# yifita/iso-points

Measured on AMD Instinct MI355X. Metric: Mpoints/s full iso-point cycle (project+resample+splat), 1M pts, higher is better.
Workload: dtype f32-class (split-fp16 operands, 2^-22: hidden-layer products from two fp16 parts per f32 operand under exact power-of-two scales, 3 fp16-MFMA passes, f32 accumulate; everything else f32)

## Files before the change

### include/isopoints.h

```cpp
#ifndef ISOPOINTS_H_
#define ISOPOINTS_H_

#include <stdint.h>

#ifdef __cplusplus
extern "C" {
#endif

#define ISO_OK 0
#define ISO_ERR_INVALID (-1)
#define ISO_ERR_UNSUPPORTED (-2)
#define ISO_ERR_LAUNCH (-3)
#define ISO_ERR_WORKSPACE (-4)

const char* iso_version(void);
const char* iso_last_error(void);


int iso_project_sphere(const float* pts_in, float* pts_out, float* normals_out,
                       uint8_t* mask_out, int64_t n, float cx, float cy,
                       float cz, float radius, int max_iters, float tol,
                       void* stream);

typedef struct iso_follow {
  void* grid_ws; int64_t grid_n_max;
  const float* views; int n_views; float znear; float zfar; int backface_culling;
  int32_t* mask_out; void* front_ws; int64_t front_ws_bytes;
  int64_t* first_idx_out; int64_t* num_pts_out; int32_t* view_total_out;
} iso_follow;

int iso_project_sphere_follow(const float* pts_in, float* pts_out, float* normals_out,
                              uint8_t* mask_out, int64_t n, float cx, float cy,
                              float cz, float radius, int max_iters, float tol,
                              const iso_follow* follow_host, void* stream);

int64_t iso_siren_raw_floats(int hidden, int n_hidden);
int64_t iso_siren_packed_floats(int hidden, int n_hidden);
int iso_siren_pack_weights(const float* raw, float* packed, int hidden,
                           int n_hidden, void* stream);
int iso_siren_set_gemm_mode(int mode);
int iso_siren_get_gemm_mode(void);
int iso_siren_set_tail_from(int first_tail_iteration);
int iso_siren_set_drawn_tiles(int on);
int iso_idr_set_drawn_tiles(int on);
int iso_siren_step_launches(int hidden, int n_hidden, int max_iters);
int64_t iso_project_siren_workspace_bytes(int64_t n, int hidden, int n_hidden);
int64_t iso_project_siren_counts_offset(int64_t n, int hidden, int n_hidden);
int iso_project_siren(const float* pts_in, float* pts_out, float* normals_out,
                      uint8_t* mask_out, int64_t n, const float* packed,
                      int hidden, int n_hidden, float omega_first,
                      float omega_hidden, int max_iters, float tol,
                      void* workspace, int64_t workspace_bytes, void* stream);
int iso_siren_sdf_grad(const float* pts, float* sdf_out, float* grad_out,
                       int64_t n, const float* packed, int hidden,
                       int n_hidden, float omega_first, float omega_hidden,
                       void* workspace, int64_t workspace_bytes, void* stream);

int iso_siren_fold_codes(const float* w0c, const float* b0, const float* codes, float* table, int hidden,
                         int padded_hidden, int c_dim, int64_t n_codes, void* stream);
int iso_project_siren_coded(const float* pts_in, float* pts_out, float* normals_out,
                            uint8_t* mask_out, int64_t n, const float* packed,
                            int hidden, int n_hidden, float omega_first,
                            float omega_hidden, int max_iters, float tol,
                            void* workspace, int64_t workspace_bytes, void* stream,
                            const float* code_bias, const int32_t* code_of, int64_t n_codes);
int iso_siren_sdf_grad_coded(const float* pts, float* sdf_out, float* grad_out,
                             int64_t n, const float* packed, int hidden,
                             int n_hidden, float omega_first, float omega_hidden,
                             void* workspace, int64_t workspace_bytes, void* stream,
                             const float* code_bias, const int32_t* code_of, int64_t n_codes);

int64_t iso_idr_raw_floats(int hidden, int n_layers, int skip_layer, int n_freq);
int64_t iso_idr_packed_floats(int hidden, int n_layers);
int iso_idr_pack_weights(const float* raw, float* packed, int hidden, int n_layers,
                         int skip_layer, int n_freq, void* stream);
int64_t iso_project_idr_workspace_bytes(int64_t n, int hidden, int n_layers);
int iso_project_idr(const float* pts_in, float* pts_out, float* normals_out, uint8_t* mask_out,
                    int64_t n, const float* packed, int hidden, int n_layers, int skip_layer,
                    int n_freq, float beta, int max_iters, float tol, void* workspace,
                    int64_t workspace_bytes, void* stream);
int iso_idr_sdf_grad(const float* pts, float* sdf_out, float* grad_out, int64_t n,
                     const float* packed, int hidden, int n_layers, int skip_layer, int n_freq,
                     float beta, void* workspace, int64_t workspace_bytes, void* stream);

int iso_trace_sphere(const float* ray0, const float* dirs, float* pts_out, float* sdf_out,
                     uint8_t* mask_out, int64_t n, float cx, float cy, float cz, float radius,
                     float alpha, float bound, int max_iters, float tol, void* stream);
int iso_trace_siren(const float* ray0, const float* dirs, float* pts_out, float* sdf_out,
                    uint8_t* mask_out, int64_t n, const float* packed, int hidden, int n_hidden,
                    float omega_first, float omega_hidden, float alpha, float bound, int max_iters,
                    float tol, void* workspace, int64_t workspace_bytes, void* stream);
int iso_trace_siren_coded(const float* ray0, const float* dirs, float* pts_out, float* sdf_out,
// ... 352 lines not shown
```

### iso_points_amd/_lib.py

```python
import ctypes
import os

import torch

_HERE = os.path.dirname(os.path.abspath(__file__))
LIB_PATH = os.path.join(_HERE, "libisopoints_hip.so")
if os.environ.get("ISO_DEV_LIB"):
    LIB_PATH = os.path.abspath(os.environ["ISO_DEV_LIB"])

_c = ctypes
_P = _c.c_void_p
_I = _c.c_int
_L = _c.c_int64
_F = _c.c_float

SIGNATURES = {
    "iso_version": (_c.c_char_p, []),
    "iso_last_error": (_c.c_char_p, []),
    "iso_project_sphere": (_I, [_P, _P, _P, _P, _L, _F, _F, _F, _F, _I, _F, _P]),
    "iso_project_sphere_follow": (_I, [_P, _P, _P, _P, _L, _F, _F, _F, _F, _I, _F, _P, _P]),
    "iso_siren_raw_floats": (_L, [_I, _I]),
    "iso_siren_packed_floats": (_L, [_I, _I]),
    "iso_siren_set_gemm_mode": (_I, [_I]),
    "iso_siren_get_gemm_mode": (_I, []),
    "iso_siren_set_tail_from": (_I, [_I]),
    "iso_siren_set_drawn_tiles": (_I, [_I]),
    "iso_idr_set_drawn_tiles": (_I, [_I]),
    "iso_siren_step_launches": (_I, [_I, _I, _I]),
    "iso_siren_pack_weights": (_I, [_P, _P, _I, _I, _P]),
    "iso_project_siren_workspace_bytes": (_L, [_L, _I, _I]),
    "iso_project_siren_counts_offset": (_L, [_L, _I, _I]),
    "iso_project_siren": (_I, [_P, _P, _P, _P, _L, _P, _I, _I, _F, _F, _I, _F, _P, _L, _P]),
    "iso_siren_sdf_grad": (_I, [_P, _P, _P, _L, _P, _I, _I, _F, _F, _P, _L, _P]),
    "iso_idr_raw_floats": (_L, [_I, _I, _I, _I]),
    "iso_idr_packed_floats": (_L, [_I, _I]),
    "iso_idr_pack_weights": (_I, [_P, _P, _I, _I, _I, _I, _P]),
    "iso_project_idr_workspace_bytes": (_L, [_L, _I, _I]),
    "iso_project_idr": (_I, [_P, _P, _P, _P, _L, _P, _I, _I, _I, _I, _F, _I, _F, _P, _L, _P]),
    "iso_idr_sdf_grad": (_I, [_P, _P, _P, _L, _P, _I, _I, _I, _I, _F, _P, _L, _P]),
    "iso_trace_sphere": (_I, [_P, _P, _P, _P, _P, _L, _F, _F, _F, _F, _F, _F, _I, _F, _P]),
    "iso_trace_siren": (_I, [_P, _P, _P, _P, _P, _L, _P, _I, _I, _F, _F, _F, _F, _I, _F, _P, _L, _P]),
    "iso_siren_fold_codes": (_I, [_P, _P, _P, _P, _I, _I, _I, _L, _P]),
    "iso_project_siren_coded": (_I, [_P, _P, _P, _P, _L, _P, _I, _I, _F, _F, _I, _F, _P, _L, _P, _P, _P, _L]),
    "iso_siren_sdf_grad_coded": (_I, [_P, _P, _P, _L, _P, _I, _I, _F, _F, _P, _L, _P, _P, _P, _L]),
    "iso_trace_siren_coded": (_I, [_P, _P, _P, _P, _P, _L, _P, _I, _I, _F, _F, _F, _F, _I, _F, _P, _L, _P, _P, _P, _L]),
    "iso_trace_idr": (_I, [_P, _P, _P, _P, _P, _L, _P, _I, _I, _I, _I, _F, _F, _F, _I, _F, _P, _L, _P]),
    "iso_ray_nearest_point_workspace_bytes": (_L, [_L]),
    "iso_ray_nearest_point": (_I, [_P, _L, _F, _F, _F, _P, _L, _P, _P, _P, _P, _L, _P]),
    "iso_raymarch_settle": (_I, [_P, _P, _L, _P, _P, _P, _P, _F, _I, _I, _P, _P, _P, _P]),
    "iso_raymarch_overshoot": (_I, [_P, _P, _L, _P, _P, _P, _P, _I, _I, _F, _P, _P, _P, _P]),
    "iso_raymarch_secant": (_I, [_P, _P, _L, _P, _P, _P, _P, _P, _P, _P, _P]),
    "iso_image_sample": (_I, [_P, _I, _I, _I, _I, _P, _L, _I, _P, _P]),
    "iso_ear_candidates": (_I, [_P, _P, _P, _P, _L, _I, _F, _P, _P, _P]),
    "iso_points_bbox": (_I, [_P, _P, _I, _L, _P, _P]),
    "iso_frnn_make_grid": (_I, [_P, _P, _P, _I, _L, _I, _P, _P]),
    "iso_frnn_make_grid_density": (_I, [_P, _P, _P, _I, _L, _I, _F, _P, _P]),
    "iso_frnn_insert_points": (_I, [_P, _P, _P, _P, _P, _P, _I, _L, _L, _I, _P]),
    "iso_prefix_sum_workspace_bytes": (_L, [_L, _I]),
    "iso_prefix_sum": (_I, [_P, _P, _L, _I, _L, _P, _L, _P]),
    "iso_frnn_scan_cells": (_I, [_P, _P, _P, _I, _L, _I, _P, _L, _P]),
    "iso_frnn_counting_sort": (_I, [_P, _P, _P, _P, _P, _P, _P, _I, _L, _L, _I, _P]),
    "iso_frnn_query_workspace_bytes": (_L, [_I, _L, _L]),
    "iso_frnn_query": (_I, [_P, _P, _P, _P, _P, _P, _P, _P, _P, _I, _P, _P, _P, _I, _L, _L, _L, _P, _L, _P]),
    "iso_frnn_gather": (_I, [_P, _P, _P, _I, _L, _L, _I, _I, _P]),
    "iso_repulse": (_I, [_P, _P, _P, _L, _P, _L, _L, _I, _P, _P]),
    "iso_upsample_candidates": (_I, [_P, _P, _L, _I, _P, _P, _P]),
    "iso_farthest_point_sampling_work_floats": (_L, [_I, _L]),
    "iso_farthest_point_sampling": (_I, [_P, _P, _P, _P, _I, _L, _L, _P, _P, _P]),
    "iso_pca_frames_work_bytes": (_L, [_I]),
    "iso_pca_frames": (_I, [_P, _P, _P, _I, _L, _I, _I, _P, _P, _P, _P]),
    "iso_splat_view_flags": (_I, [_P, _P, _P, _P, _L, _I, _F, _F, _I, _P]),
    "iso_compact_rows": (_I, [_P, _P, _P, _P, _L, _L, _I, _P]),
    "iso_splat_vrk_h": (_I, [_P, _P, _P, _P, _P, _I, _L, _P]),
    "iso_splat_setup": (_I, [_P, _P, _P, _P, _P, _P, _P, _I, _L, _I, _F, _F, _P, _P, _P, _P, _P, _P]),
    "iso_splat_vrk_h_global_work_bytes": (_L, [_I]),
    "iso_splat_vrk_h_global": (_I, [_P, _P, _P, _P, _I, _L, _L, _P, _P]),
    "iso_splat_tangent_frame": (_I, [_P, _L, _P, _P, _P]),
    "iso_splat_setup_vrk": (_I, [_P, _P, _P, _P, _P, _P, _P, _I, _L, _I, _F, _F, _P, _P, _P, _P, _P, _P]),
    "iso_splat_setup_aniso": (_I, [_P, _P, _L, _P, _P, _P, _P, _I, _I, _F, _F, _P, _P, _P, _P, _P, _P]),
    "iso_splat_tiles_per_side": (_I, [_I]),
    "iso_splat_bin_count": (_I, [_P, _P, _P, _P, _I, _L, _I, _I, _I, _I, _P, _P]),
    "iso_splat_tile_offsets": (_I, [_P, _P, _P, _L, _P]),
# ... 121 lines not shown
```

### iso_points_amd/csrc/siren.hip

```cpp
#include <stdlib.h>
#include "siren_common.h"
#include "iso_newton.h"
#include "mlp_common.h"

namespace {

__global__ void k_siren_pack(const float* __restrict__ raw, float* __restrict__ packed,
                             int H, int L) {
  const int64_t total = off_hidden(H, L);
  const int64_t HH = (int64_t)H * H;
  const int NT = H / 16;
  for (int64_t o = (int64_t)blockIdx.x * blockDim.x + threadIdx.x; o < total;
       o += (int64_t)gridDim.x * blockDim.x) {
    float v = 0.f;
    if (o < off_wl(H)) {
      int64_t k = o;
      int c = (int)(k & 3);
      int e = (int)((k >> 2) % (H / 4));
      int g = (int)((k >> 2) / (H / 4));
      int f = 16 * (e >> 2) + 4 * g + (e & 3);
      v = (c < 3) ? raw[f * 3 + c] : raw[(int64_t)H * 3 + f];
    } else if (o < off_bl(H)) {
      int64_t k = o - off_wl(H);
      int e = (int)(k % (H / 4));
      int g = (int)(k / (H / 4));
      int f = 16 * (e >> 2) + 4 * g + (e & 3);
      const int64_t raw_wl = (int64_t)H * 4 + (int64_t)L * (HH + H);
      v = raw[raw_wl + f];
    } else if (o < off_hidden(H, 0)) {
      const int64_t raw_wl = (int64_t)H * 4 + (int64_t)L * (HH + H);
      v = (o == off_bl(H)) ? raw[raw_wl + H] : 0.f;
    } else {
      int64_t k = o - off_hidden(H, 0);
      const int64_t per = H + 2 * HH;
      int l = (int)(k / per);
      int64_t w = k % per;
      const float* Wl = raw + (int64_t)H * 4 + (int64_t)l * (HH + H);
      const float* bl = Wl + HH;
      if (w < H) {
        v = bl[w];
      } else {
        w -= H;
        bool bwd = w >= HH;
        if (bwd) w -= HH;
        int i = (int)(w & 3);
        int lane = (int)((w >> 2) & 63);
        int t = (int)((w >> 8) % NT);
        int q = (int)((w >> 8) / NT);
        int a = 16 * t + (lane & 15);
        int b = 16 * q + 4 * (lane >> 4) + i;
        v = bwd ? Wl[(int64_t)b * H + a]
                : Wl[(int64_t)a * H + b];
      }
    }
    packed[o] = v;
  }
}

#define ISO_GEMM_FWD(img, bias) gemm_pass<NT, true>(img, bias, hL, wbuf, acc, lane, g)
#define ISO_GEMM_BWD(img) gemm_pass<NT, false>(img, nullptr, hL, wbuf, acc, lane, g)

template <int NT, bool CODED>
__global__ __launch_bounds__(256, 2) void k_siren_step(typename SirenArgsOf<CODED>::type a) {
  constexpr int H = NT * 16;
  extern __shared__ __attribute__((aligned(16))) float smem[];
  const int tid = threadIdx.x;
  const int wave = tid >> 6, lane = tid & 63;
  const int g = lane >> 4, j = lane & 15;
  float* hL = smem + wave * (NT * 256);
  float* wbuf = smem + 4 * NT * 256;
  const float* W0img = a.packed + off_w0(H);
  const float* WLimg = a.packed + off_wl(H);
  const float bL = a.packed[off_bl(H)];
  float* stash = a.stash + ((int64_t)blockIdx.x * 4 + wave) * (int64_t)(a.L + 1) * NT * 256;

  const int64_t count = a.count_in ? (int64_t)(*a.count_in) : a.n;
  const int64_t n_tiles = (count + 63) / 64;
  for (int64_t tile = blockIdx.x; tile < n_tiles; tile += gridDim.x) {
    const int64_t slot = tile * 64 + wave * 16 + j;
    const bool valid = slot < count;
    int64_t idx = -1;
    float px = 0.f, py = 0.f, pz = 0.f;
    int row = 0;
    if (valid) {
      idx = a.idx_in ? (int64_t)a.idx_in[slot] : slot;
      px = a.pts[idx * 3]; py = a.pts[idx * 3 + 1]; pz = a.pts[idx * 3 + 2];
      if constexpr (CODED) row = a.code_of ? a.code_of[idx] : 0;
    }
    const f32x4* cb = nullptr;
    if constexpr (CODED) cb = reinterpret_cast<const f32x4*>(a.code_bias + (int64_t)row * H) + g;
    (void)cb;
    float f = 0.f;
    const bool top0 = (a.L == 0);
    for (int e4 = 0; e4 < NT; ++e4) {
      f32x4 h4, s4;
      f32x4 b4 = {0.f, 0.f, 0.f, 0.f};
      if constexpr (CODED) b4 = cb[4 * e4];
#pragma unroll
      for (int i = 0; i < 4; ++i) {
        const f32x4 w = reinterpret_cast<const f32x4*>(W0img)[g * (H / 4) + e4 * 4 + i];
        float z;
        if constexpr (CODED) z = ((w.x * px + w.y * py) + w.z * pz) + b4[i];
        else z = ((w.x * px + w.y * py) + w.z * pz) + w.w;
        float s, c;
        iso_sincos(a.w0 * z, s, c);
        h4[i] = s;
        s4[i] = a.w0 * c;
      }
      if (top0) {
// ... 109 lines not shown
}

__global__ void k_zero_counts(int32_t* c, int n) {
  int i = blockIdx.x * blockDim.x + threadIdx.x;
  if (i < n) c[i] = 0;
}

bool siren_shape_ok(int H, int L) {
  return (H == 64 || H == 128 || H == 256) && L >= 0 && L <= 8;
}

int g_gemm_mode = -1;
int gemm_mode() {
  if (g_gemm_mode < 0) {
    const char* e = getenv("ISO_SIREN_GEMM");
    g_gemm_mode = (e && (!strcmp(e, "f32") || !strcmp(e, "0"))) ? 0 : 1;
  }
  return g_gemm_mode;
}
bool use_x3(int H, int L) { return gemm_mode() == 1 && siren_x3_supported(H, L); }

int64_t stash_floats_any(int H, int L) {
  int64_t a = stash_floats(H, L);
  int64_t b = siren_x3_supported(H, L) ? siren_x3_stash_floats(H, L) : 0;
  return a > b ? a : b;
}

int run_step(const SirenCodedArgs& a, int H, int64_t n, hipStream_t s) {
  if (use_x3(H, a.L)) return siren_x3_launch(a, H, n, s);
  int64_t tiles = (n + 63) / 64;
  int blocks = (int)(tiles < kSirenBlocks ? tiles : kSirenBlocks);
  return a.code_bias ? dispatch_step<true>(a, H, blocks, s) : dispatch_step<false>(a, H, blocks, s);
}

}

extern "C" int64_t iso_siren_raw_floats(int hidden, int n_hidden) {
  int64_t H = hidden;
  return H * 3 + H + (int64_t)n_hidden * (H * H + H) + H + 1;
}

extern "C" int64_t iso_siren_packed_floats(int hidden, int n_hidden) {
  return siren_packed_total(hidden, n_hidden);
}

extern "C" int iso_siren_set_gemm_mode(int mode) {
  ISO_REQUIRE(mode == 0 || mode == 1, ISO_ERR_INVALID, "iso_siren_set_gemm_mode: mode must be 0 (f32 MFMA) or 1 (split fp16)");
  g_gemm_mode = mode;
  return ISO_OK;
}

extern "C" int iso_siren_get_gemm_mode(void) { return gemm_mode(); }

extern "C" int iso_siren_pack_weights(const float* raw, float* packed, int hidden,
                                      int n_hidden, void* stream) {
  ISO_REQUIRE(siren_shape_ok(hidden, n_hidden), ISO_ERR_UNSUPPORTED,
              "iso_siren_pack_weights: hidden must be 64/128/256 and 0<=n_hidden<=8 (got %d, %d)",
              hidden, n_hidden);
  ISO_REQUIRE(raw && packed, ISO_ERR_INVALID, "iso_siren_pack_weights: null pointer");
  int64_t total = off_hidden(hidden, n_hidden);
  hipLaunchKernelGGL(k_siren_pack, dim3(iso_stream_grid(total, 256)), dim3(256), 0,
                     (hipStream_t)stream, raw, packed, hidden, n_hidden);
  if (hidden % 32 == 0) siren_x3_pack(raw, packed, hidden, n_hidden, (hipStream_t)stream);
  ISO_CHECK_LAUNCH("iso_siren_pack_weights");
  return ISO_OK;
}

static int64_t tail_cap_of(int64_t n) {
  const int64_t blocks = siren_x3_tail_blocks(), tiles = (n + 31) / 32;
  return ((tiles + blocks - 1) / blocks + 1) * 32;
}
static int64_t tail_ints(int64_t n) { return siren_x3_tail_blocks() * (2 * tail_cap_of(n) + 2); }

constexpr int kTileCtrInts = 128;
extern "C" int64_t iso_project_siren_workspace_bytes(int64_t n, int hidden, int n_hidden) {
  if (n < 0) n = 0;
  return stash_floats_any(hidden, n_hidden) * 4 + 2 * n * 4 + tail_ints(n) * 4 + (64 + kTileCtrInts) * 4 + 64;
}

extern "C" int64_t iso_project_siren_counts_offset(int64_t n, int hidden, int n_hidden) {
  if (n < 0) n = 0;
  return stash_floats_any(hidden, n_hidden) * 4 + 2 * n * 4 + tail_ints(n) * 4;
}

static int g_siren_dyn_tiles = -1;
static bool siren_dynamic_tiles_enabled() {
  return g_siren_dyn_tiles != 0;
}
extern "C" int iso_siren_set_drawn_tiles(int on) {
  ISO_REQUIRE(on >= -1 && on <= 1, ISO_ERR_INVALID, "iso_siren_set_drawn_tiles: -1 (default), 0 or 1");
  g_siren_dyn_tiles = on;
  return ISO_OK;
}

static int run_step_split(SirenCodedArgs a, int hidden, int64_t n, hipStream_t s) {
  if (hidden == 256 && !a.fwd_only && use_x3(hidden, a.L)) {
    a.split = 3;
    return run_step(a, hidden, n, s);
  }
  a.split = 0;
  a.tile_ctr = nullptr;
  return run_step(a, hidden, n, s);
}

static int g_tail_from = -1;
static int siren_tail_from(int max_iters) {
  if (g_tail_from == 0) return max_iters + 1;
  if (g_tail_from > 0) return g_tail_from;
  return max_iters >= 6 ? 4 : 2;
}
extern "C" int iso_siren_step_launches(int hidden, int n_hidden, int max_iters) {
  if (max_iters < 0) return 0;
  const bool can_tail = hidden == 256 && use_x3(hidden, n_hidden);
  const int from = can_tail ? siren_tail_from(max_iters) : max_iters + 1;
  return from <= max_iters && from > 0 ? from + 1 : max_iters + 1;
}
// ... 236 lines not shown
```

### iso_points_amd/csrc/siren_common.h

```cpp
#pragma once
#include "iso_common.h"

struct SirenArgs {
  float* pts;
  float* normals;
  uint8_t* mask;
  float* sdf_out;
  float* grad_out;
  const int32_t* idx_in;
  const int32_t* count_in;
  int32_t* idx_out;
  int32_t* count_out;
  const float* packed;
  float* stash;
  int64_t n;
  int L;
  float w0, wh, tol;
  int do_move;
  int eval_only;
  const float* dirs = nullptr;
  float alpha = 1.f, bound = 0.f, tol_valid = 0.f;
  int fwd_only = 0;
  int64_t cnt_lo = -1, cnt_hi = INT64_MAX;
  int small_tiles = 0;
  int split = 0;
  int big_blocks = 0;
  int32_t* tail_lists = nullptr;
  int32_t* tail_counts = nullptr;
  int32_t* iter_counts = nullptr;
  int tail_cap = 0, it_first = 0, it_last = 0;
  int32_t* tile_ctr = nullptr;
  int draw_first = 0;
  int ps_guard = 0;
};

struct SirenCodedArgs : SirenArgs {
  const float* code_bias = nullptr;
  const int32_t* code_of = nullptr;
};
template <bool CODED> struct SirenArgsOf { using type = SirenArgs; };
template <> struct SirenArgsOf<true> { using type = SirenCodedArgs; };

__host__ __device__ inline int64_t siren_split_point(int64_t count) {
  const int64_t big = 256 * 96, small = 256 * 32;
  const int64_t full = count / big * big, rem = count - full;
  if (rem == 0) return count;
  return (rem + small - 1) / small <= 2 ? full : count;
}

__host__ __device__ inline int64_t off_w0(int H) { (void)H; return 0; }
__host__ __device__ inline int64_t off_wl(int H) { return 4 * (int64_t)H; }
__host__ __device__ inline int64_t off_bl(int H) { return 5 * (int64_t)H; }
__host__ __device__ inline int64_t off_hidden(int H, int l) {
  return 5 * (int64_t)H + 4 + (int64_t)l * ((int64_t)H + 2 * (int64_t)H * H);
}

__host__ __device__ inline int x3_feat(int s, int kappa) {
  return 32 * (s >> 1) + 16 * (s & 1) + 8 * ((kappa & 7) >> 2) + 4 * (kappa >> 3) + (kappa & 3);
}
__host__ __device__ inline int64_t x3_base(int H, int L) { return off_hidden(H, L); }
__host__ __device__ inline int64_t x3_off_w0(int H, int L) { return x3_base(H, L); }
__host__ __device__ inline int64_t x3_off_wl(int H, int L) { return x3_base(H, L) + 4 * (int64_t)H; }
__host__ __device__ inline int64_t x3_off_layer(int H, int L, int l) {
  return x3_base(H, L) + 5 * (int64_t)H + (int64_t)l * (int64_t)H;
}
constexpr int kX16Header = 24;
__host__ __device__ inline int64_t x16_base(int H, int L) { return x3_off_layer(H, L, L); }
__host__ __device__ inline int64_t x16_off_layer(int H, int L, int l) { return x16_base(H, L) + kX16Header + (int64_t)l * H * H; }
__host__ __device__ inline int64_t x16_off_bw(int H, int L, int l) { return x16_off_layer(H, L, L) + (int64_t)l * H * H; }
__host__ __device__ inline int64_t siren_packed_total(int H, int L) { return x16_off_bw(H, L, L); }

bool siren_x3_supported(int H, int L);
int64_t siren_x3_stash_floats(int H, int L);
void siren_x3_pack(const float* raw, float* packed, int H, int L, hipStream_t s);
int siren_x3_launch(const SirenCodedArgs& a, int H, int64_t n_upper, hipStream_t s);
int siren_x3_tail_blocks();
int siren_x3_launch_tail(const SirenCodedArgs& a, int H, hipStream_t s);
constexpr int64_t kPsMinList = 3 * 256 * 128;
__host__ __device__ inline bool siren_ps_takes(int64_t count, int L, const float* hdr , float wh) {
  if (count < kPsMinList) return false;
  float r = 0.f;
  for (int l = 0; l < L; ++l) r = hdr[17 + l] > r ? hdr[17 + l] : r;
  return (wh * r) * 1.01f < 1.0e4f;
}
```

### iso_points_amd/csrc/siren_x3.hip

```cpp
#include <stdlib.h>
#include <type_traits>
#include "siren_common.h"
#include "iso_newton.h"
#include "mlp_common.h"

#include "mfma_split.h"

constexpr int kAD = 3;

namespace {

__device__ __forceinline__ void x3_sin_wcos8(float w_in, float w, const float (&z)[8], float (&s)[8], float (&c)[8]) {
  iso_sin_wcos8(w_in, w, z, s, c);
}


__global__ void k_siren_pack_x3(const float* __restrict__ raw, float* __restrict__ packed, int H, int L) {
  const int64_t base = x3_base(H, L), total = x16_base(H, L);
  const int64_t HH = (int64_t)H * H;
  const float* b0 = raw + (int64_t)H * 3;
  const float* WL = raw + (int64_t)H * 4 + (int64_t)L * (HH + H);
  for (int64_t o = base + (int64_t)blockIdx.x * blockDim.x + threadIdx.x; o < total;
       o += (int64_t)gridDim.x * blockDim.x) {
    const int64_t rel = o - base;
    auto feat_of = [](int64_t ko) { return x3_feat((int)(ko >> 4), 8 * (int)((ko >> 3) & 1) + (int)(ko & 7)); };
    if (rel < 4 * (int64_t)H) {
      const int f = feat_of(rel >> 2), c = (int)(rel & 3);
      packed[o] = (c < 3) ? raw[f * 3 + c] : b0[f];
    } else if (rel < 5 * (int64_t)H) {
      packed[o] = WL[feat_of(rel - 4 * (int64_t)H)];
    } else {
      const int64_t r2 = rel - 5 * (int64_t)H;
      const int l = (int)(r2 / H);
      const float* Wl = raw + (int64_t)H * 4 + (int64_t)l * (HH + H);
      packed[o] = Wl[HH + feat_of(r2 % H)];
    }
  }
}

__global__ void k_siren_wscale(const float* __restrict__ raw, float* __restrict__ packed, int H, int L) {
  __shared__ float s_m[256];
  const int l = blockIdx.x;
  const int64_t HH = (int64_t)H * H;
  const float* Wl = raw + (int64_t)H * 4 + (int64_t)l * (HH + H);
  float m = 0.f, cs = 0.f;
  for (int f = threadIdx.x; f < H; f += 256) {
    float t = 0.f;
#pragma unroll 32
    for (int k = 0; k < H; ++k) {
      const float a = fabsf(Wl[(int64_t)k * H + f]);
      m = (a == a && a > m) ? a : m;
      t += a;
    }
    cs = fmaxf(cs, t);
  }
  s_m[threadIdx.x] = m;
  __syncthreads();
  for (int o = 128; o > 0; o >>= 1) {
    if ((int)threadIdx.x < o) s_m[threadIdx.x] = fmaxf(s_m[threadIdx.x], s_m[threadIdx.x + o]);
    __syncthreads();
  }
  if (threadIdx.x == 0) {
    float mx = s_m[0];
    int e = 0;
    float sc = 1.0f;
    if (mx > 0.f && mx < 3.0e38f) {
      (void)frexpf(mx, &e);
      int k = 10 - e;
      k = k > 100 ? 100 : (k < -100 ? -100 : k);
      sc = ldexpf(1.0f, k);
    }
    packed[x16_base(H, L) + l] = sc;
  }
  __syncthreads();
  s_m[threadIdx.x] = cs;
  __syncthreads();
  for (int o = 128; o > 0; o >>= 1) {
    if ((int)threadIdx.x < o) s_m[threadIdx.x] = fmaxf(s_m[threadIdx.x], s_m[threadIdx.x + o]);
    __syncthreads();
  }
  if (threadIdx.x == 0) packed[x16_base(H, L) + 8 + l] = s_m[0];
  if (l == 0) {
    __syncthreads();
    const float* WLh = raw + (int64_t)H * 4 + (int64_t)L * (HH + H);
    float mh = 0.f;
    for (int f = threadIdx.x; f < H; f += 256) mh = fmaxf(mh, fabsf(WLh[f]));
    s_m[threadIdx.x] = mh;
    __syncthreads();
    for (int o = 128; o > 0; o >>= 1) {
      if ((int)threadIdx.x < o) s_m[threadIdx.x] = fmaxf(s_m[threadIdx.x], s_m[threadIdx.x + o]);
      __syncthreads();
    }
    if (threadIdx.x == 0) packed[x16_base(H, L) + 16] = s_m[0];
  }
}

__global__ void k_siren_pack_f16(const float* __restrict__ raw, float* __restrict__ packed, int H, int L) {
  const int64_t HH = (int64_t)H * H;
  const int NTO = H / 32;
  const int64_t total = 2 * (int64_t)L * HH;
  for (int64_t o = (int64_t)blockIdx.x * blockDim.x + threadIdx.x; o < total; o += (int64_t)gridDim.x * blockDim.x) {
    const bool bwd = o >= (int64_t)L * HH;
    const int l = (int)((o / HH) % L);
    const int64_t q = o % HH;
    const float* Wl = raw + (int64_t)H * 4 + (int64_t)l * (HH + H);
    const float sc = packed[x16_base(H, L) + l];
    const int d = (int)(q & 3), lane = (int)((q >> 2) & 63);
    const int64_t blk = q >> 8;
    const int part = (int)(blk & 1);
    const int To = (int)((blk >> 1) % NTO), s = (int)(blk / (2 * NTO));
    const int fo = 32 * To + (lane & 31);
    f32x2 v;
#pragma unroll
    for (int u = 0; u < 2; ++u) {
      const int fi = x3_feat(s, 8 * (lane >> 5) + 2 * d + u);
      v[u] = (bwd ? Wl[(int64_t)fi * H + fo] : Wl[(int64_t)fo * H + fi]) * sc;
    }
    const f16x2 h = __builtin_convertvector(v, f16x2);
    const f16x2 lo = __builtin_convertvector(v - __builtin_convertvector(h, f32x2), f16x2);
    reinterpret_cast<unsigned*>(packed + x16_off_layer(H, L, 0))[o] =
        part == 0 ? __builtin_bit_cast(unsigned, h) : __builtin_bit_cast(unsigned, lo);
  }
}

template <int H, int NW, int NB>
struct X3Shape {
  static constexpr int NS = H / 16;
  static constexpr int NTO = H / 32;
  static constexpr int TW = NTO / NW;
  static constexpr int SL = 2 * TW;
  static constexpr int NG = SL * NB;
  static constexpr int P = 32 * NB;
  static constexpr size_t kActBytes = (size_t)NS * NB * kAP * 1024;
  static constexpr size_t kRedBytes = (size_t)NW * P * 16;
  static constexpr size_t kPtsBytes = (size_t)P * 16;
  static constexpr int kLdsGroupsFit = (int)((163840 - (kActBytes + kRedBytes + kPtsBytes)) / ((size_t)NW * 2048));
  static constexpr int LG = kLdsGroupsFit < NG ? kLdsGroupsFit : NG;
  static constexpr size_t kLds = kActBytes + kRedBytes + kPtsBytes + (size_t)NW * LG * 2048;
  static constexpr int64_t kStashPerWg(int L) { return (int64_t)NW * (L > 1 ? L : 1) * NG * 512; }
  static_assert(NTO % NW == 0 && TW >= 1, "features must split evenly over the waves");
};

template <int H>
__device__ __forceinline__ void x3_code_bias8(const float* table, int row, int s, int h, float (&b)[8]) {
  const f32x4* t = reinterpret_cast<const f32x4*>(table + (int64_t)row * H + 16 * s + 4 * h);
  const f32x4 lo = t[0], hi = t[2];
#pragma unroll
  for (int e = 0; e < 4; ++e) { b[e] = lo[e]; b[4 + e] = hi[e]; }
}

template <int H, int NW, int NB, bool FWD, bool CODED>
__device__ __forceinline__ void x3_step_body(const typename SirenArgsOf<CODED>::type& a, const int bid, const int nblk,
                                             const int sid) {
  using S = X3Shape<H, NW, NB>;
  constexpr int NS = S::NS, NTO = S::NTO, TW = S::TW, SL = S::SL, NG = S::NG, P = S::P;
  extern __shared__ __attribute__((aligned(16))) unsigned char smem_raw[];
  u32x4* act = reinterpret_cast<u32x4*>(smem_raw);
  f32x4* red = reinterpret_cast<f32x4*>(smem_raw + S::kActBytes);
  f32x4* ptl = reinterpret_cast<f32x4*>(smem_raw + S::kActBytes + S::kRedBytes);
  constexpr int LG = S::LG;
  const int tid = threadIdx.x;
  const int w = __builtin_amdgcn_readfirstlane(tid >> 6);
  const int lane = tid & 63, h = lane >> 5, j = lane & 31;
  u32x4* own = act + (size_t)(SL * w) * NB * kAP * 64 + lane;
  u32x4* park = own + (size_t)(kAP - 2) * NG * 64;
  constexpr bool IL = (NW == 8);
  const int L = a.L;
  const float* X = a.packed + x3_base(H, L);
  const f32x4* W0u = reinterpret_cast<const f32x4*>(X) + SL * w * 16;
  const float* WLu = X + 4 * H + SL * w * 16;
  const int h8 = h * 8;
  const float bL = a.packed[off_bl(H)];
  f32x4* stash = reinterpret_cast<f32x4*>(a.stash) +
                 ((int64_t)sid * NW + w) * (int64_t)(L > 1 ? L : 1) * NG * 128;
  f32x4* lst = reinterpret_cast<f32x4*>(smem_raw + S::kActBytes + S::kRedBytes + S::kPtsBytes) + w * (LG * 128) + lane;
// ... 441 lines not shown
}

template <int H, int NW, int NB, int MINB, bool FWD, bool CODED>
int launch_x3(const typename SirenArgsOf<CODED>::type& a, int64_t n_upper, hipStream_t s) {
  using S = X3Shape<H, NW, NB>;
  static bool attr_done = false;
  if (!attr_done) {
    (void)hipFuncSetAttribute(reinterpret_cast<const void*>(&k_siren_step_x3<H, NW, NB, MINB, FWD, CODED>),
                              hipFuncAttributeMaxDynamicSharedMemorySize, (int)S::kLds);
    attr_done = true;
  }
  const int64_t tiles = (n_upper + S::P - 1) / S::P;
  const int64_t cap = 256 * MINB;
  const int blocks = (int)(tiles < cap ? (tiles < 1 ? 1 : tiles) : cap);
  hipLaunchKernelGGL((k_siren_step_x3<H, NW, NB, MINB, FWD, CODED>), dim3(blocks), dim3(64 * NW), S::kLds, s, a);
  return 0;
}

template <int H, int NW, int NB, int MINB, bool CODED>
int launch_x3_both(typename SirenArgsOf<CODED>::type a, int64_t n_upper, hipStream_t s) {
  using SB = X3Shape<H, NW, NB>;
  using SS = X3Shape<H, NW, 1>;
  constexpr size_t lds = SB::kLds > SS::kLds ? SB::kLds : SS::kLds;
  static bool attr_done = false;
  if (!attr_done) {
    (void)hipFuncSetAttribute(reinterpret_cast<const void*>(&k_siren_step_x3_both<H, NW, NB, MINB, CODED>),
                              hipFuncAttributeMaxDynamicSharedMemorySize, (int)lds);
    attr_done = true;
  }
  const int64_t cap = 256 * MINB;
  const int64_t tb = (n_upper + SB::P - 1) / SB::P, ts = (n_upper + SS::P - 1) / SS::P;
  a.big_blocks = (int)(tb < cap ? (tb < 1 ? 1 : tb) : cap);
  const int small_blocks = (int)(ts < cap ? (ts < 1 ? 1 : ts) : cap);
  hipLaunchKernelGGL((k_siren_step_x3_both<H, NW, NB, MINB, CODED>), dim3(a.big_blocks + small_blocks), dim3(64 * NW), lds, s, a);
  return 0;
}

}

constexpr int kNW256 = 8;
constexpr int kMinB256 = 1;
constexpr int kNB256 = 3;
constexpr int kMinB128 = 1;
bool siren_x3_supported(int H, int L) { return (H == 256 || H == 128) && L >= 1 && L <= 8; }

int64_t siren_x3_stash_floats(int H, int L) {
  if (H == 256) {
    return 256 * kMinB256 * (X3Shape<256, kNW256, kNB256>::kStashPerWg(L) + X3Shape<256, kNW256, 1>::kStashPerWg(L));
  }
  if (H == 128) return 256 * kMinB128 * X3Shape<128, 4, 3>::kStashPerWg(L);
  return 0;
}

void siren_x3_pack(const float* raw, float* packed, int H, int L, hipStream_t s) {
  const int64_t words = x16_base(H, L) - x3_base(H, L);
  hipLaunchKernelGGL(k_siren_pack_x3, dim3(iso_stream_grid(words, 256)), dim3(256), 0, s, raw, packed, H, L);
  if (L > 0) {
    hipLaunchKernelGGL(k_siren_wscale, dim3(L), dim3(256), 0, s, raw, packed, H, L);
    hipLaunchKernelGGL(k_siren_pack_f16, dim3(iso_stream_grid(2 * (int64_t)L * H * H, 256)), dim3(256), 0, s, raw, packed, H, L);
  }
}

int siren_x3_tail_blocks() { return 256 * kMinB256; }

template <bool CODED>
static int launch_tail(const typename SirenArgsOf<CODED>::type& a, hipStream_t s) {
  using SS = X3Shape<256, kNW256, 1>;
  static bool attr_done = false;
  if (!attr_done) {
    (void)hipFuncSetAttribute(reinterpret_cast<const void*>(&k_siren_tail_x3<256, kNW256, kMinB256, CODED>),
                              hipFuncAttributeMaxDynamicSharedMemorySize, (int)SS::kLds);
    attr_done = true;
  }
  hipLaunchKernelGGL((k_siren_tail_x3<256, kNW256, kMinB256, CODED>), dim3(siren_x3_tail_blocks()), dim3(64 * kNW256), SS::kLds, s, a);
  return 0;
}

int siren_x3_launch_tail(const SirenCodedArgs& a, int H, hipStream_t s) {
  if (H != 256) return -1;
  return a.code_bias ? launch_tail<true>(a, s) : launch_tail<false>(a, s);
}

template <bool CODED>
static int launch_any(const typename SirenArgsOf<CODED>::type& a, int H, int64_t n_upper, hipStream_t s) {
  if (a.split == 3 && H == 256 && !a.fwd_only) return launch_x3_both<256, kNW256, kNB256, kMinB256, CODED>(a, n_upper, s);
  if (a.fwd_only) {
    if (H == 256) return launch_x3<256, kNW256, kNB256, kMinB256, true, CODED>(a, n_upper, s);
    if (H == 128) return launch_x3<128, 4, 3, kMinB128, true, CODED>(a, n_upper, s);
  }
  if constexpr (!CODED) {
    if (H == 256) return launch_x3<256, kNW256, kNB256, kMinB256, false, false>(a, n_upper, s);
  }
  if (H == 128) return launch_x3<128, 4, 3, kMinB128, false, CODED>(a, n_upper, s);
  return -1;
}

int siren_x3_launch(const SirenCodedArgs& a, int H, int64_t n_upper, hipStream_t s) {
  return a.code_bias ? launch_any<true>(a, H, n_upper, s) : launch_any<false>(a, H, n_upper, s);
}
```

Before: 76.26.

## Fuse SIREN weight packing kernels into a single launch

```diff
diff --git a/include/isopoints.h b/include/isopoints.h
--- a/include/isopoints.h
+++ b/include/isopoints.h
@@ -38,6 +38,7 @@
 int64_t iso_siren_packed_floats(int hidden, int n_hidden);
 int iso_siren_pack_weights(const float* raw, float* packed, int hidden,
                            int n_hidden, void* stream);
+int iso_siren_set_pack_fused(int on);
 int iso_siren_set_gemm_mode(int mode);
 int iso_siren_get_gemm_mode(void);
 int iso_siren_set_tail_from(int first_tail_iteration);
diff --git a/iso_points_amd/_lib.py b/iso_points_amd/_lib.py
--- a/iso_points_amd/_lib.py
+++ b/iso_points_amd/_lib.py
@@ -28,6 +28,7 @@
     "iso_idr_set_drawn_tiles": (_I, [_I]),
     "iso_siren_step_launches": (_I, [_I, _I, _I]),
     "iso_siren_pack_weights": (_I, [_P, _P, _I, _I, _P]),
+    "iso_siren_set_pack_fused": (_I, [_I]),
     "iso_project_siren_workspace_bytes": (_L, [_L, _I, _I]),
     "iso_project_siren_counts_offset": (_L, [_L, _I, _I]),
     "iso_project_siren": (_I, [_P, _P, _P, _P, _L, _P, _I, _I, _F, _F, _I, _F, _P, _L, _P]),
diff --git a/iso_points_amd/csrc/siren.hip b/iso_points_amd/csrc/siren.hip
--- a/iso_points_amd/csrc/siren.hip
+++ b/iso_points_amd/csrc/siren.hip
@@ -7,54 +7,7 @@
 
 __global__ void k_siren_pack(const float* __restrict__ raw, float* __restrict__ packed,
                              int H, int L) {
-  const int64_t total = off_hidden(H, L);
-  const int64_t HH = (int64_t)H * H;
-  const int NT = H / 16;
-  for (int64_t o = (int64_t)blockIdx.x * blockDim.x + threadIdx.x; o < total;
-       o += (int64_t)gridDim.x * blockDim.x) {
-    float v = 0.f;
-    if (o < off_wl(H)) {
-      int64_t k = o;
-      int c = (int)(k & 3);
-      int e = (int)((k >> 2) % (H / 4));
-      int g = (int)((k >> 2) / (H / 4));
-      int f = 16 * (e >> 2) + 4 * g + (e & 3);
-      v = (c < 3) ? raw[f * 3 + c] : raw[(int64_t)H * 3 + f];
-    } else if (o < off_bl(H)) {
-      int64_t k = o - off_wl(H);
-      int e = (int)(k % (H / 4));
-      int g = (int)(k / (H / 4));
-      int f = 16 * (e >> 2) + 4 * g + (e & 3);
-      const int64_t raw_wl = (int64_t)H * 4 + (int64_t)L * (HH + H);
-      v = raw[raw_wl + f];
-    } else if (o < off_hidden(H, 0)) {
-      const int64_t raw_wl = (int64_t)H * 4 + (int64_t)L * (HH + H);
-      v = (o == off_bl(H)) ? raw[raw_wl + H] : 0.f;
-    } else {
-      int64_t k = o - off_hidden(H, 0);
-      const int64_t per = H + 2 * HH;
-      int l = (int)(k / per);
-      int64_t w = k % per;
-      const float* Wl = raw + (int64_t)H * 4 + (int64_t)l * (HH + H);
-      const float* bl = Wl + HH;
-      if (w < H) {
-        v = bl[w];
-      } else {
-        w -= H;
-        bool bwd = w >= HH;
-        if (bwd) w -= HH;
-        int i = (int)(w & 3);
-        int lane = (int)((w >> 2) & 63);
-        int t = (int)((w >> 8) % NT);
-        int q = (int)((w >> 8) / NT);
-        int a = 16 * t + (lane & 15);
-        int b = 16 * q + 4 * (lane >> 4) + i;
-        v = bwd ? Wl[(int64_t)b * H + a]
-                : Wl[(int64_t)a * H + b];
-      }
-    }
-    packed[o] = v;
-  }
+  siren_pack_f32(raw, packed, H, L, (int64_t)blockIdx.x * blockDim.x + threadIdx.x, (int64_t)gridDim.x * blockDim.x);
 }
 
 #define ISO_GEMM_FWD(img, bias) gemm_pass<NT, true>(img, bias, hL, wbuf, acc, lane, g)
@@ -270,16 +223,28 @@
 
 extern "C" int iso_siren_get_gemm_mode(void) { return gemm_mode(); }
 
+static int g_siren_pack_fused = -1;
+extern "C" int iso_siren_set_pack_fused(int on) {
+  ISO_REQUIRE(on >= -1 && on <= 1, ISO_ERR_INVALID, "iso_siren_set_pack_fused: -1 (default), 0 or 1");
+  g_siren_pack_fused = on;
+  return ISO_OK;
+}
+
 extern "C" int iso_siren_pack_weights(const float* raw, float* packed, int hidden,
                                       int n_hidden, void* stream) {
   ISO_REQUIRE(siren_shape_ok(hidden, n_hidden), ISO_ERR_UNSUPPORTED,
               "iso_siren_pack_weights: hidden must be 64/128/256 and 0<=n_hidden<=8 (got %d, %d)",
               hidden, n_hidden);
   ISO_REQUIRE(raw && packed, ISO_ERR_INVALID, "iso_siren_pack_weights: null pointer");
-  int64_t total = off_hidden(hidden, n_hidden);
-  hipLaunchKernelGGL(k_siren_pack, dim3(iso_stream_grid(total, 256)), dim3(256), 0,
-                     (hipStream_t)stream, raw, packed, hidden, n_hidden);
-  if (hidden % 32 == 0) siren_x3_pack(raw, packed, hidden, n_hidden, (hipStream_t)stream);
+  const bool fused = hidden % 32 == 0 && g_siren_pack_fused != 0;
+  if (fused) {
+    siren_x3_pack(raw, packed, hidden, n_hidden, true, (hipStream_t)stream);
+  } else {
+    int64_t total = off_hidden(hidden, n_hidden);
+    hipLaunchKernelGGL(k_siren_pack, dim3(iso_stream_grid(total, 256)), dim3(256), 0,
+                       (hipStream_t)stream, raw, packed, hidden, n_hidden);
+    if (hidden % 32 == 0) siren_x3_pack(raw, packed, hidden, n_hidden, false, (hipStream_t)stream);
+  }
   ISO_CHECK_LAUNCH("iso_siren_pack_weights");
   return ISO_OK;
 }
diff --git a/iso_points_amd/csrc/siren_common.h b/iso_points_amd/csrc/siren_common.h
--- a/iso_points_amd/csrc/siren_common.h
+++ b/iso_points_amd/csrc/siren_common.h
@@ -70,9 +70,60 @@
 __host__ __device__ inline int64_t x16_off_bw(int H, int L, int l) { return x16_off_layer(H, L, L) + (int64_t)l * H * H; }
 __host__ __device__ inline int64_t siren_packed_total(int H, int L) { return x16_off_bw(H, L, L); }
 
+__device__ inline void siren_pack_f32(const float* __restrict__ raw, float* __restrict__ packed, int H, int L,
+                                      int64_t first, int64_t stride) {
+  const int64_t total = off_hidden(H, L);
+  const int64_t HH = (int64_t)H * H;
+  const int NT = H / 16;
+  for (int64_t o = first; o < total; o += stride) {
+    float v = 0.f;
+    if (o < off_wl(H)) {
+      int64_t k = o;
+      int c = (int)(k & 3);
+      int e = (int)((k >> 2) % (H / 4));
+      int g = (int)((k >> 2) / (H / 4));
+      int f = 16 * (e >> 2) + 4 * g + (e & 3);
+      v = (c < 3) ? raw[f * 3 + c] : raw[(int64_t)H * 3 + f];
+    } else if (o < off_bl(H)) {
+      int64_t k = o - off_wl(H);
+      int e = (int)(k % (H / 4));
+      int g = (int)(k / (H / 4));
+      int f = 16 * (e >> 2) + 4 * g + (e & 3);
+      const int64_t raw_wl = (int64_t)H * 4 + (int64_t)L * (HH + H);
+      v = raw[raw_wl + f];
+    } else if (o < off_hidden(H, 0)) {
+      const int64_t raw_wl = (int64_t)H * 4 + (int64_t)L * (HH + H);
+      v = (o == off_bl(H)) ? raw[raw_wl + H] : 0.f;
+    } else {
+      int64_t k = o - off_hidden(H, 0);
+      const int64_t per = H + 2 * HH;
+      int l = (int)(k / per);
+      int64_t w = k % per;
+      const float* Wl = raw + (int64_t)H * 4 + (int64_t)l * (HH + H);
+      const float* bl = Wl + HH;
+      if (w < H) {
+        v = bl[w];
+      } else {
+        w -= H;
+        bool bwd = w >= HH;
+        if (bwd) w -= HH;
+        int i = (int)(w & 3);
+        int lane = (int)((w >> 2) & 63);
+        int t = (int)((w >> 8) % NT);
+        int q = (int)((w >> 8) / NT);
+        int a = 16 * t + (lane & 15);
+        int b = 16 * q + 4 * (lane >> 4) + i;
+        v = bwd ? Wl[(int64_t)b * H + a]
+                : Wl[(int64_t)a * H + b];
+      }
+    }
+    packed[o] = v;
+  }
+}
+
 bool siren_x3_supported(int H, int L);
 int64_t siren_x3_stash_floats(int H, int L);
-void siren_x3_pack(const float* raw, float* packed, int H, int L, hipStream_t s);
+void siren_x3_pack(const float* raw, float* packed, int H, int L, bool with_f32, hipStream_t s);
 int siren_x3_launch(const SirenCodedArgs& a, int H, int64_t n_upper, hipStream_t s);
 int siren_x3_tail_blocks();
 int siren_x3_launch_tail(const SirenCodedArgs& a, int H, hipStream_t s);
diff --git a/iso_points_amd/csrc/siren_x3.hip b/iso_points_amd/csrc/siren_x3.hip
--- a/iso_points_amd/csrc/siren_x3.hip
+++ b/iso_points_amd/csrc/siren_x3.hip
@@ -15,13 +15,13 @@
 }
 
 
-__global__ void k_siren_pack_x3(const float* __restrict__ raw, float* __restrict__ packed, int H, int L) {
+__device__ void x3_pack_korder(const float* __restrict__ raw, float* __restrict__ packed, int H, int L, int64_t first,
+                               int64_t stride) {
   const int64_t base = x3_base(H, L), total = x16_base(H, L);
   const int64_t HH = (int64_t)H * H;
   const float* b0 = raw + (int64_t)H * 3;
   const float* WL = raw + (int64_t)H * 4 + (int64_t)L * (HH + H);
-  for (int64_t o = base + (int64_t)blockIdx.x * blockDim.x + threadIdx.x; o < total;
-       o += (int64_t)gridDim.x * blockDim.x) {
+  for (int64_t o = base + first; o < total; o += stride) {
     const int64_t rel = o - base;
     auto feat_of = [](int64_t ko) { return x3_feat((int)(ko >> 4), 8 * (int)((ko >> 3) & 1) + (int)(ko & 7)); };
     if (rel < 4 * (int64_t)H) {
@@ -38,9 +38,31 @@
   }
 }
 
-__global__ void k_siren_wscale(const float* __restrict__ raw, float* __restrict__ packed, int H, int L) {
-  __shared__ float s_m[256];
-  const int l = blockIdx.x;
+__device__ __forceinline__ float x3_weight_scale(float mx) {
+  int e = 0;
+  float sc = 1.0f;
+  if (mx > 0.f && mx < 3.0e38f) {
+    (void)frexpf(mx, &e);
+    int k = 10 - e;
+    k = k > 100 ? 100 : (k < -100 ? -100 : k);
+    sc = ldexpf(1.0f, k);
+  }
+  return sc;
+}
+
+__device__ __forceinline__ float x3_block_max(float v, float* s_m) {
+  s_m[threadIdx.x] = v;
+  __syncthreads();
+  for (int o = 128; o > 0; o >>= 1) {
+    if ((int)threadIdx.x < o) s_m[threadIdx.x] = fmaxf(s_m[threadIdx.x], s_m[threadIdx.x + o]);
+    __syncthreads();
+  }
+  const float r = s_m[0];
+  __syncthreads();
+  return r;
+}
+
+__device__ void x3_wscale_layer(const float* __restrict__ raw, float* __restrict__ packed, int H, int L, int l, float* s_m) {
   const int64_t HH = (int64_t)H * H;
   const float* Wl = raw + (int64_t)H * 4 + (int64_t)l * (HH + H);
   float m = 0.f, cs = 0.f;
@@ -54,73 +76,89 @@
     }
     cs = fmaxf(cs, t);
   }
-  s_m[threadIdx.x] = m;
-  __syncthreads();
-  for (int o = 128; o > 0; o >>= 1) {
-    if ((int)threadIdx.x < o) s_m[threadIdx.x] = fmaxf(s_m[threadIdx.x], s_m[threadIdx.x + o]);
-    __syncthreads();
-  }
-  if (threadIdx.x == 0) {
-    float mx = s_m[0];
-    int e = 0;
-    float sc = 1.0f;
-    if (mx > 0.f && mx < 3.0e38f) {
-      (void)frexpf(mx, &e);
-      int k = 10 - e;
-      k = k > 100 ? 100 : (k < -100 ? -100 : k);
-      sc = ldexpf(1.0f, k);
-    }
-    packed[x16_base(H, L) + l] = sc;
-  }
-  __syncthreads();
-  s_m[threadIdx.x] = cs;
-  __syncthreads();
-  for (int o = 128; o > 0; o >>= 1) {
-    if ((int)threadIdx.x < o) s_m[threadIdx.x] = fmaxf(s_m[threadIdx.x], s_m[threadIdx.x + o]);
-    __syncthreads();
-  }
-  if (threadIdx.x == 0) packed[x16_base(H, L) + 8 + l] = s_m[0];
+  const float mx = x3_block_max(m, s_m);
+  if (threadIdx.x == 0) packed[x16_base(H, L) + l] = x3_weight_scale(mx);
+  const float c = x3_block_max(cs, s_m);
+  if (threadIdx.x == 0) packed[x16_base(H, L) + 8 + l] = c;
   if (l == 0) {
-    __syncthreads();
     const float* WLh = raw + (int64_t)H * 4 + (int64_t)L * (HH + H);
     float mh = 0.f;
     for (int f = threadIdx.x; f < H; f += 256) mh = fmaxf(mh, fabsf(WLh[f]));
-    s_m[threadIdx.x] = mh;
-    __syncthreads();
-    for (int o = 128; o > 0; o >>= 1) {
-      if ((int)threadIdx.x < o) s_m[threadIdx.x] = fmaxf(s_m[threadIdx.x], s_m[threadIdx.x + o]);
-      __syncthreads();
-    }
-    if (threadIdx.x == 0) packed[x16_base(H, L) + 16] = s_m[0];
-  }
+    const float h = x3_block_max(mh, s_m);
+    if (threadIdx.x == 0) packed[x16_base(H, L) + 16] = h;
+  }
+}
+
+__device__ __forceinline__ void x3_pack_f16_word(const float* __restrict__ raw, float* __restrict__ packed, int H, int L,
+                                                 int64_t o, int l, float sc) {
+  const int64_t HH = (int64_t)H * H;
+  const int NTO = H / 32;
+  const bool bwd = o >= (int64_t)L * HH;
+  const int64_t q = o % HH;
+  const float* Wl = raw + (int64_t)H * 4 + (int64_t)l * (HH + H);
+  const int d = (int)(q & 3), lane = (int)((q >> 2) & 63);
+  const int64_t blk = q >> 8;
+  const int part = (int)(blk & 1);
+  const int To = (int)((blk >> 1) % NTO), s = (int)(blk / (2 * NTO));
+  const int fo = 32 * To + (lane & 31);
+  f32x2 v;
+#pragma unroll
+  for (int u = 0; u < 2; ++u) {
+    const int fi = x3_feat(s, 8 * (lane >> 5) + 2 * d + u);
+    v[u] = (bwd ? Wl[(int64_t)fi * H + fo] : Wl[(int64_t)fo * H + fi]) * sc;
+  }
+  const f16x2 h = __builtin_convertvector(v, f16x2);
+  const f16x2 lo = __builtin_convertvector(v - __builtin_convertvector(h, f32x2), f16x2);
+  reinterpret_cast<unsigned*>(packed + x16_off_layer(H, L, 0))[o] =
+      part == 0 ? __builtin_bit_cast(unsigned, h) : __builtin_bit_cast(unsigned, lo);
+}
+
+__global__ void k_siren_pack_x3(const float* __restrict__ raw, float* __restrict__ packed, int H, int L) {
+  x3_pack_korder(raw, packed, H, L, (int64_t)blockIdx.x * blockDim.x + threadIdx.x, (int64_t)gridDim.x * blockDim.x);
+}
+
+__global__ __launch_bounds__(256) void k_siren_wscale(const float* __restrict__ raw, float* __restrict__ packed, int H, int L) {
+  __shared__ float s_m[256];
+  x3_wscale_layer(raw, packed, H, L, blockIdx.x, s_m);
 }
 
 __global__ void k_siren_pack_f16(const float* __restrict__ raw, float* __restrict__ packed, int H, int L) {
   const int64_t HH = (int64_t)H * H;
-  const int NTO = H / 32;
   const int64_t total = 2 * (int64_t)L * HH;
   for (int64_t o = (int64_t)blockIdx.x * blockDim.x + threadIdx.x; o < total; o += (int64_t)gridDim.x * blockDim.x) {
-    const bool bwd = o >= (int64_t)L * HH;
     const int l = (int)((o / HH) % L);
-    const int64_t q = o % HH;
+    x3_pack_f16_word(raw, packed, H, L, o, l, packed[x16_base(H, L) + l]);
+  }
+}
+
+constexpr int kX16Chunk = 4096;
+__global__ __launch_bounds__(256) void k_siren_pack_fused(const float* __restrict__ raw, float* __restrict__ packed, int H,
+                                                          int L, int n_img, int with_f32) {
+  __shared__ float s_m[256];
+  const int bid = blockIdx.x;
+  if (bid < L) { x3_wscale_layer(raw, packed, H, L, bid, s_m); return; }
+  if (bid < L + n_img) {
+    const int64_t HH = (int64_t)H * H;
+    const int64_t o0 = (int64_t)(bid - L) * kX16Chunk;
+    const int l = (int)((o0 / HH) % L);
     const float* Wl = raw + (int64_t)H * 4 + (int64_t)l * (HH + H);
-    const float sc = packed[x16_base(H, L) + l];
-    const int d = (int)(q & 3), lane = (int)((q >> 2) & 63);
-    const int64_t blk = q >> 8;
-    const int part = (int)(blk & 1);
-    const int To = (int)((blk >> 1) % NTO), s = (int)(blk / (2 * NTO));
-    const int fo = 32 * To + (lane & 31);
-    f32x2 v;
-#pragma unroll
-    for (int u = 0; u < 2; ++u) {
-      const int fi = x3_feat(s, 8 * (lane >> 5) + 2 * d + u);
-      v[u] = (bwd ? Wl[(int64_t)fi * H + fo] : Wl[(int64_t)fo * H + fi]) * sc;
-    }
-    const f16x2 h = __builtin_convertvector(v, f16x2);
-    const f16x2 lo = __builtin_convertvector(v - __builtin_convertvector(h, f32x2), f16x2);
-    reinterpret_cast<unsigned*>(packed + x16_off_layer(H, L, 0))[o] =
-        part == 0 ? __builtin_bit_cast(unsigned, h) : __builtin_bit_cast(unsigned, lo);
-  }
+    float m = 0.f;
+    auto take = [&m](float x) { const float a = fabsf(x); m = (a == a && a > m) ? a : m; };
+    if (((uintptr_t)Wl & 15) == 0) {
+      const f32x4* W4 = reinterpret_cast<const f32x4*>(Wl);
+#pragma unroll 16
+      for (int i = threadIdx.x; i < (int)(HH / 4); i += 256) { const f32x4 w = W4[i]; take(w[0]); take(w[1]); take(w[2]); take(w[3]); }
+    } else {
+#pragma unroll 16
+      for (int i = threadIdx.x; i < (int)HH; i += 256) take(Wl[i]);
+    }
+    const float sc = x3_weight_scale(x3_block_max(m, s_m));
+    for (int64_t o = o0 + threadIdx.x; o < o0 + kX16Chunk; o += 256) x3_pack_f16_word(raw, packed, H, L, o, l, sc);
+    return;
+  }
+  const int64_t first = (int64_t)(bid - L - n_img) * 256 + threadIdx.x, stride = (int64_t)((int)gridDim.x - L - n_img) * 256;
+  if (with_f32) siren_pack_f32(raw, packed, H, L, first, stride);
+  x3_pack_korder(raw, packed, H, L, first, stride);
 }
 
 template <int H, int NW, int NB>
@@ -668,8 +706,14 @@
   return 0;
 }
 
-void siren_x3_pack(const float* raw, float* packed, int H, int L, hipStream_t s) {
+void siren_x3_pack(const float* raw, float* packed, int H, int L, bool with_f32, hipStream_t s) {
   const int64_t words = x16_base(H, L) - x3_base(H, L);
+  if (with_f32) {
+    const int n_img = (int)(2 * (int64_t)L * H * H / kX16Chunk);
+    const int n_rest = iso_stream_grid(off_hidden(H, L) > words ? off_hidden(H, L) : words, 256);
+    hipLaunchKernelGGL(k_siren_pack_fused, dim3(L + n_img + n_rest), dim3(256), 0, s, raw, packed, H, L, n_img, 1);
+    return;
+  }
   hipLaunchKernelGGL(k_siren_pack_x3, dim3(iso_stream_grid(words, 256)), dim3(256), 0, s, raw, packed, H, L);
   if (L > 0) {
     hipLaunchKernelGGL(k_siren_wscale, dim3(L), dim3(256), 0, s, raw, packed, H, L);
```

After: 76.50, median of 3. No clear change (+0.3%).
